# JuliaRobotics/RigidBodyDynamics.jl

Measured on AMD Instinct MI355X. Metric: ABA dynamics! evals/sec (Atlas 30-DoF, batch), higher is better.
Workload: dtype f64

## Files before the change

### rigidbodydynamics.jl_amd/csrc/rbd_bank.hpp

```cpp
#pragma once

#ifndef RBD_BANK_WAVES
#define RBD_BANK_WAVES 2
#endif
#ifndef RBD_BANK_FK_LDS
#define RBD_BANK_FK_LDS 0
#endif
#ifndef RBD_BANK_HANDOFF_LDS
#define RBD_BANK_HANDOFF_LDS 0
#endif

#ifdef RBD_BANK_FIXED_NL
#define RBD_BANK_UNROLL _Pragma("unroll")
namespace rbd { constexpr int kBankNs[] = {RBD_BANK_FIXED_NS}; }
#define RBD_BK_NL RBD_BANK_FIXED_NL
#define RBD_BK_L0 RBD_BANK_FIXED_L0
#define RBD_BK_NS(l) kBankNs[l]
#ifdef RBD_BANK_FIXED_PERM
#define RBD_BK_PERM(l) (((RBD_BANK_FIXED_PERM) >> (l)) & 1ull)
#else
#define RBD_BK_PERM(l) (kBankNs[l] > 1)
#endif
#else
#define RBD_BANK_UNROLL _Pragma("unroll 1")
#define RBD_BK_NL M.nlevels
#define RBD_BK_L0 M.L0
#define RBD_BK_NS(l) ns_next(nss, M.ns_desc)
#define RBD_BK_PERM(l) ((M.perm_down >> (l)) & 1)
#endif

namespace rbd {

template <typename T> struct alignas(2 * sizeof(T)) Pair2 { T a, b; };

RBD_DEV void wave_lds_sync() {
  __builtin_amdgcn_fence(__ATOMIC_RELEASE, "wavefront");
  __builtin_amdgcn_wave_barrier();
  __builtin_amdgcn_fence(__ATOMIC_ACQUIRE, "wavefront");
}


#define RBD_MASSIGN6(MOV)                                                                                                              \
  unsigned long long sv;                                                                                                               \
  asm volatile("s_and_saveexec_b64 %[sv], %[mk]\n\t" MOV " %[d0], %[s0]\n\t" MOV " %[d1], %[s1]\n\t" MOV " %[d2], %[s2]\n\t" MOV          \
               " %[d3], %[s3]\n\t" MOV " %[d4], %[s4]\n\t" MOV " %[d5], %[s5]\n\ts_mov_b64 exec, %[sv]\n\ts_nop 0"                         \
               : [sv] "=&s"(sv), [d0] "+v"(d[0]), [d1] "+v"(d[1]), [d2] "+v"(d[2]), [d3] "+v"(d[3]), [d4] "+v"(d[4]), [d5] "+v"(d[5])    \
               : [mk] "s"(mask), [s0] "v"(s[0]), [s1] "v"(s[1]), [s2] "v"(s[2]), [s3] "v"(s[3]), [s4] "v"(s[4]), [s5] "v"(s[5])          \
               : "scc")
RBD_DEV void massign6(unsigned long long mask, double* d, const double* s) { RBD_MASSIGN6("v_mov_b64"); }
RBD_DEV void massign6(unsigned long long mask, float* d, const float* s) { RBD_MASSIGN6("v_mov_b32"); }
template <typename T, int N> RBD_DEV void massign(bool m, T* d, const T* s) {
  static_assert(N % 6 == 0, "blocks of 6");
  const unsigned long long mask = __builtin_amdgcn_ballot_w64(m);
#pragma unroll
  for (int k = 0; k < N; k += 6) massign6(mask, d + k, s + k);
}

enum { PK_KIN = 0, PK_FWD = 6, PARK_PAIRS = 16, PK_XCH = 16, XCH_PAIRS = 14, BANK_LDS_PAIRS = PARK_PAIRS + XCH_PAIRS };

template <typename T, int N> RBD_DEV void lds_put(Pair2<T>* col, int pair0, const T* x) {
#pragma unroll
  for (int i = 0; i < (N + 1) / 2; ++i) {
    Pair2<T> v;
    v.a = x[2 * i];
    v.b = (2 * i + 1 < N) ? x[2 * i + 1] : T(0);
    col[(pair0 + i) * 256] = v;
  }
}
template <typename T, int N> RBD_DEV void lds_get(const Pair2<T>* col, int pair0, T* x) {
#pragma unroll
  for (int i = 0; i < (N + 1) / 2; ++i) {
    const Pair2<T> v = col[(pair0 + i) * 256];
    x[2 * i] = v.a;
    if (2 * i + 1 < N) x[2 * i + 1] = v.b;
  }
}

__host__ __device__ constexpr int sym_row(int e) { return e < 6 ? 0 : e < 11 ? 1 : e < 15 ? 2 : e < 18 ? 3 : e < 20 ? 4 : 5; }
__host__ __device__ constexpr int sym_col(int e) { return e - SI(sym_row(e), sym_row(e)) + sym_row(e); }

template <typename T> struct BankRegs {
  Body<T> b;
  const T* rb;
  int pcol;
  T K[24];
  RBD_DEV T* R() { return K; }
  RBD_DEV T* p() { return K + 9; }
  RBD_DEV T* Tw() { return K + 12; }
  RBD_DEV T* vJ() { return K + 18; }
  T S[6], cb[6], IA[21], pA[6], U[6], Dinv, u;
  T tj[6];
  T acc[6], vd[6];
};

template <typename T> RBD_DEV void load_bank_body(const BankModel& M, int k, long B, Body<T>& b) {
  const int tid = blockIdx.x * blockDim.x + threadIdx.x;
  b.lane = threadIdx.x & 63;
  const long wave = tid >> 6;
  const int lps = M.lps;
  b.sub = b.lane & (lps - 1);
  b.base = b.lane - b.sub;
  b.state = wave * (64 / lps) + (b.lane / lps);
  b.valid = (b.sub < M.nbk[k]) && (b.state < B);
  const int4* ib4 = reinterpret_cast<const int4*>(M.ib[k] + (b.sub < M.nbk[k] ? b.sub : 0) * IB_STRIDE);
  const int4 w0 = ib4[0], w1 = ib4[1], w2 = ib4[2], w3 = ib4[3];
  static_assert(IB_PARENT == 0 && IB_JTYPE == 1 && IB_QOFF == 2 && IB_VOFF == 3 && IB_LEVEL == 4 && IB_NCHILD == 5 && IB_ORIG == 6 && IB_CHILD0 == 7 &&
                IB_MAXCHILD == 8 && IB_FLAGS == 15 && IB_STRIDE == 16, "record layout");
  b.parent = w0.x; b.jtype = w0.y; b.qoff = w0.z; b.voff = w0.w;
  b.level = b.valid ? w1.x : -1;
  b.nchild = w1.y; b.orig = w1.z;
  b.child[0] = w1.w; b.child[1] = w2.x; b.child[2] = w2.y; b.child[3] = w2.z; b.child[4] = w2.w; b.child[5] = w3.x; b.child[6] = w3.y; b.child[7] = w3.z;
  b.flags = w3.w;
  b.plane = b.parent >= 0 ? b.base + b.parent : b.lane;
}

template <typename T, bool SIMPLE>
RBD_DEV void bank_fk_commit(bool mine, BankRegs<T>& c, const T* k18 , const T* XR, const T* Xp, const T* tl) {
  const T* pR = k18;
  const T* pp = k18 + 9;
  const T* pT = k18 + 12;
  T n[24];
  matmul3(pR, XR, n);
  matvec3(pR, Xp, n + 9);
#pragma unroll
  for (int k = 0; k < 3; ++k) n[9 + k] += pp[k];
  if (SIMPLE) {
    T S[6];
    matvec3(n, tl, S);
    cross3(n + 9, S, S + 3);
#pragma unroll
    for (int k = 0; k < 6; ++k) n[12 + k] = pT[k] + S[k] * tl[3];
    massign<T, 18>(mine, c.K, n);
  } else {
    xmotion(n, n + 9, tl, n + 18);
#pragma unroll
    for (int k = 0; k < 6; ++k) n[12 + k] = pT[k] + n[18 + k];
    massign<T, 24>(mine, c.K, n);
  }
}
template <typename T, bool SIMPLE> RBD_DEV void bank_fk_step(const BankModel& M, int l, bool perm, BankRegs<T>& c, Pair2<T>* lds, const T* XR, const T* Xp, const T* tl) {
  T k18[18];
  if (RBD_BANK_FK_LDS || perm) {
    if (c.b.level == l - 1 && c.b.nchild >= 1) {
      RBD_KEEP_BRANCH();
      lds_put<T, 18>(lds + threadIdx.x, PK_XCH, c.K);
    }
    wave_lds_sync();
    lds_get<T, 18>(lds + c.pcol, PK_XCH, k18);
    wave_lds_sync();
  } else {
#pragma unroll
    for (int k = 0; k < 18; ++k) k18[k] = from_prev_lane(c.K[k]);
  }
  bank_fk_commit<T, SIMPLE>(c.b.level == l, c, k18, XR, Xp, tl);
}
template <typename T, bool SIMPLE> RBD_DEV void bank_fk_cross(int L0, BankRegs<T>& c, const Pair2<T>* lds, const T* XR, const T* Xp, const T* tl) {
  T k18[18];
  lds_get<T, 18>(lds + c.pcol, PK_KIN, k18);
  bank_fk_commit<T, SIMPLE>(c.b.level == L0, c, k18, XR, Xp, tl);
}

// ... 69 lines not shown
        for (int k = 0; k < 6; ++k) tk.pA[k] += x[21 + k];
      }
    }
    wave_lds_sync();
  }
}

template <typename T> RBD_DEV void bank_joint_accel(bool mine, BankRegs<T>& r, const T* a_parent) {
  T ap[6], n[6];
#pragma unroll
  for (int k = 0; k < 6; ++k) ap[k] = a_parent[k] + r.cb[k];
  const T x = r.Dinv * (r.u - dot6(r.U, ap));
#pragma unroll
  for (int k = 0; k < 6; ++k) n[k] = ap[k] + r.S[k] * x;
  massign<T, 6>(mine, r.acc, n);
  r.vd[0] = mine ? x : r.vd[0];
}
template <typename T> RBD_DEV void bank_accel_step(const BankModel& M, int l, bool perm, BankRegs<T>& c, Pair2<T>* lds) {
  T ap[6];
  if (RBD_BANK_FK_LDS || perm) {
    if (c.b.level == l - 1 && c.b.nchild >= 1) {
      RBD_KEEP_BRANCH();
      lds_put<T, 6>(lds + threadIdx.x, PK_XCH, c.acc);
    }
    wave_lds_sync();
    lds_get<T, 6>(lds + c.pcol, PK_XCH, ap);
    wave_lds_sync();
  } else {
#pragma unroll
    for (int k = 0; k < 6; ++k) ap[k] = from_prev_lane(c.acc[k]);
  }
  bank_joint_accel(c.b.level == l, c, ap);
}

#ifdef RBD_PROFILE_PHASES
__device__ long long rbd_bank_phase_clock[16];
#define RBD_MARK(i) do { if (blockIdx.x == 0 && threadIdx.x == 0) rbd_bank_phase_clock[i] = clock64(); } while (0)
#else
#define RBD_MARK(i)
#endif

template <typename T, bool R> struct InPtr { typedef const T* type; };
template <typename T> struct InPtr<T, true> { typedef const T* __restrict__ type; };

template <typename T, bool FUSED, bool SIMPLE>
RBD_DEV void aba_bank_body(const BankModel& M, long B, typename InPtr<T, !FUSED>::type q, typename InPtr<T, !FUSED>::type v, const T* __restrict__ tau,
                           const T* __restrict__ fext, T* __restrict__ vdot, T* __restrict__ qdot, Layout Lq, Layout Lv, Layout Lf, const MkFuse& F,
                           Pair2<T>* const lds) {
  Pair2<T>* const col = lds + threadIdx.x;
  RBD_MARK(0);
  BankRegs<T> r0, r1;
  auto fetch = [&](int k, BankRegs<T>& c, T* qj, T* vj) {
    load_bank_body(M, k, B, c.b);
    c.rb = reinterpret_cast<const T*>(M.rb[k]) + (c.b.sub < M.nbk[k] ? c.b.sub : 0) * RB_STRIDE;
    c.pcol = (int)threadIdx.x - c.b.sub + (c.b.parent >= 0 ? c.b.parent : c.b.sub);
    if (SIMPLE) {
      const bool fl = c.b.jtype == RBD_JOINT_QUAT_FLOATING;
      const long sc = c.b.state < B ? c.b.state : B - 1;
      const T* qp = q + ((long)c.b.qoff * Lq.sk + sc * Lq.sb);
      const long va = (long)c.b.voff * Lv.sk + sc * Lv.sb;
      const bool hv = v != nullptr, ht = tau != nullptr;
      qj[0] = qp[0];
      vj[0] = hv ? v[va] : T(0);
      c.tj[0] = ht ? tau[va] : T(0);
#pragma unroll
      for (int k2 = 1; k2 < 7; ++k2) qj[k2] = T(0);
#pragma unroll
      for (int k2 = 1; k2 < 6; ++k2) { vj[k2] = T(0); c.tj[k2] = T(0); }
      if (fl) {
        RBD_KEEP_BRANCH();
#pragma unroll
        for (int k2 = 1; k2 < 7; ++k2) qj[k2] = qp[k2 * Lq.sk];
        if (hv) {
#pragma unroll
          for (int k2 = 1; k2 < 6; ++k2) vj[k2] = v[va + k2 * Lv.sk];
        }
        if (ht) {
#pragma unroll
          for (int k2 = 1; k2 < 6; ++k2) c.tj[k2] = tau[va + k2 * Lv.sk];
        }
      }
    } else {
      load_joint_q(c.b, q, Lq, qj);
      load_joint_v(c.b, v, Lv, vj);
      load_joint_v(c.b, tau, Lv, c.tj);
    }
  };
  auto setup = [&](BankRegs<T>& c, T* qj, T* vj, T* XR, T* Xp, T* tl, T* ta ) {
    if (SIMPLE) {
      const bool fl = c.b.jtype == RBD_JOINT_QUAT_FLOATING;
      const T ax[3] = {c.rb[RB_AXIS], c.rb[RB_AXIS + 1], c.rb[RB_AXIS + 2]};
      T Rj[9], pj[3] = {T(0), T(0), T(0)};
      T sn, cs;
      ta[0] = ax[0]; ta[1] = ax[1]; ta[2] = ax[2]; ta[3] = vj[0];
      sincos_fast(qj[0], &sn, &cs);
      rot_axis_sc(ax, sn, cs, Rj);
#pragma unroll
      for (int k = 0; k < 3; ++k) { tl[k] = ax[k] * vj[0]; tl[3 + k] = T(0); }
      if (fl) {
        RBD_KEEP_BRANCH();
        rot_quat(qj[0], qj[1], qj[2], qj[3], Rj);
        pj[0] = qj[4]; pj[1] = qj[5]; pj[2] = qj[6];
#pragma unroll
        for (int k = 0; k < 6; ++k) tl[k] = vj[k];
        if (qdot != nullptr && c.b.valid) {
          const T w = qj[0], x = qj[1], y = qj[2], z = qj[3];
          T o[7];
// ... 54 lines not shown
      se3_comm(c.Tw(), c.S, c.cb);
#pragma unroll
      for (int i = 0; i < 6; ++i) c.cb[i] *= c.K[18];
    } else {
      se3_comm(c.Tw(), c.vJ(), c.cb);
    }
    RInertia<T> I;
    T Jb[6], mc[3], fe[6];
#pragma unroll
    for (int i = 0; i < 6; ++i) Jb[i] = c.rb[RB_J + i];
#pragma unroll
    for (int i = 0; i < 3; ++i) mc[i] = c.rb[RB_MC + i];
    inertia_to_root(Jb, mc, c.rb[RB_M], c.R(), c.p(), I);
    T Io[21], po[6];
    sym6_from_inertia(I, Io);
    momentum_cross(I, c.Tw(), po);
    load_body_wrench(c.b, fext, Lf, fe);
#pragma unroll
    for (int i = 0; i < 21; ++i) c.IA[i] = accumulate ? c.IA[i] + Io[i] : Io[i];
#pragma unroll
    for (int i = 0; i < 6; ++i) c.pA[i] = accumulate ? c.pA[i] + (po[i] - fe[i]) : po[i] - fe[i];
#pragma unroll
    for (int i = 0; i < 6; ++i) c.U[i] = T(0);
    c.Dinv = T(0);
    c.u = T(0);
    if (floating) xforce(c.R(), c.p(), c.tj, c.U);
  };

  T qj0[7], vj0[6], qj1[7], vj1[6];
  fetch(0, r0, qj0, vj0);
  fetch(1, r1, qj1, vj1);
  if (FUSED) {
    if (F.close_prev) {
      mk_stage_lane(r0.b, 4, (T)F.dt, qj0, vj0, (const T*)nullptr, F.W, (T*)F.q_state, (T*)F.v_state, Lq, Lv);
      mk_stage_lane(r1.b, 4, (T)F.dt, qj1, vj1, (const T*)nullptr, F.W, (T*)F.q_state, (T*)F.v_state, Lq, Lv);
    }
    mk_stage_lane(r0.b, F.stage, (T)F.dt, qj0, vj0, (const T*)nullptr, F.W, (T*)F.q_state, (T*)F.v_state, Lq, Lv);
    mk_stage_lane(r1.b, F.stage, (T)F.dt, qj1, vj1, (const T*)nullptr, F.W, (T*)F.q_state, (T*)F.v_state, Lq, Lv);
    pd_control_lane(r0.b, F, Lq, qj0, vj0, r0.tj);
    pd_control_lane(r1.b, F, Lq, qj1, vj1, r1.tj);
  }
  {
    T XR[9], Xp[3], tl[6], ta[4];
    setup(r0, qj0, vj0, XR, Xp, tl, ta);
    RBD_MARK(1);
RBD_BANK_UNROLL
    for (int l = 1; l < RBD_BK_L0; ++l) bank_fk_step<T, SIMPLE>(M, l, RBD_BK_PERM(l), r0, lds, XR, Xp, SIMPLE ? ta : tl);
  }
  {
    T XR[9], Xp[3], tl[6], ta[4];
    RBD_MARK(2);
    setup(r1, qj1, vj1, XR, Xp, tl, ta);
    RBD_MARK(3);
    lds_put<T, (SIMPLE ? 20 : 24)>(col, PK_KIN, r0.K);
    wave_lds_sync();
    bank_fk_cross<T, SIMPLE>(RBD_BK_L0, r1, lds, XR, Xp, SIMPLE ? ta : tl);
RBD_BANK_UNROLL
    for (int l = RBD_BK_L0 + 1; l < RBD_BK_NL; ++l) bank_fk_step<T, SIMPLE>(M, l, RBD_BK_PERM(l), r1, lds, XR, Xp, SIMPLE ? ta : tl);
  }
  RBD_MARK(4);
  terms(r1, false);
  RBD_MARK(5);

  NsStream nss = ns_begin(M.ns_desc);
  (void)nss;
RBD_BANK_UNROLL
  for (int l = RBD_BK_NL - 1; l > RBD_BK_L0; --l) {
    bank_finish_joint<T, SIMPLE>(l, r1);
    bank_handoff<T, RBD_BANK_HANDOFF_LDS>(l, RBD_BK_NS(l), r1, r1, lds);
  }
  bank_finish_joint<T, SIMPLE>(RBD_BK_L0, r1);
  RBD_MARK(6);
#pragma unroll
  for (int i = 0; i < 21; ++i) r0.IA[i] = T(0);
#pragma unroll
  for (int i = 0; i < 6; ++i) r0.pA[i] = T(0);
  bank_handoff<T, 1>(RBD_BK_L0, RBD_BK_NS(RBD_BK_L0), r1, r0, lds);
  {
    lds_get<T, (SIMPLE ? 20 : 24)>(col, PK_KIN, r0.K);
    T f20[20];
#pragma unroll
    for (int i = 0; i < 6; ++i) { f20[i] = r1.U[i]; f20[8 + i] = r1.S[i]; f20[14 + i] = r1.cb[i]; }
    f20[6] = r1.Dinv;
    f20[7] = r1.u;
    lds_put<T, 20>(col, PK_FWD, f20);
  }
  RBD_MARK(7);
  terms(r0, true);
  RBD_MARK(8);
RBD_BANK_UNROLL
  for (int l = RBD_BK_L0 - 1; l >= 1; --l) {
    bank_finish_joint<T, SIMPLE>(l, r0);
    bank_handoff<T, RBD_BANK_HANDOFF_LDS>(l, RBD_BK_NS(l), r0, r0, lds);
  }
  bank_finish_joint<T, SIMPLE>(0, r0);
  RBD_MARK(9);

#pragma unroll
  for (int i = 0; i < 6; ++i) { r0.acc[i] = T(0); r0.vd[i] = T(0); }
  {
    const T a0[6] = {T(0), T(0), T(0), T(-M.gravity[0]), T(-M.gravity[1]), T(-M.gravity[2])};
    BankRegs<T>& c = r0;
    const bool fl0 = c.b.level == 0 && c.b.jtype == RBD_JOINT_QUAT_FLOATING;
    T fa[6] = {T(0), T(0), T(0), T(0), T(0), T(0)}, fv[6] = {T(0), T(0), T(0), T(0), T(0), T(0)};
    if (fl0) {
      RBD_KEEP_BRANCH();
      T rhs[6], d[6], k12[12];
#pragma unroll
      for (int i = 0; i < 6; ++i) rhs[i] = c.U[i] - c.pA[i];
      sym6_solve(c.IA, rhs, fa);
#pragma unroll
      for (int i = 0; i < 6; ++i) d[i] = fa[i] - a0[i];
      lds_get<T, 12>(col, PK_KIN, k12);
      xmotion_inv(k12, k12 + 9, d, fv);
    }
    massign<T, 6>(fl0, c.acc, fa);
    massign<T, 6>(fl0, c.vd, fv);
    bank_joint_accel(c.b.level == 0 && !fl0, c, a0);
  }
RBD_BANK_UNROLL
  for (int l = 1; l < RBD_BK_L0; ++l) bank_accel_step<T>(M, l, RBD_BK_PERM(l), r0, lds);
  RBD_MARK(10);
  if (vdot) store_joint_v(r0.b, vdot, Lv, r0.vd);
  if (FUSED) store_joint_v(r0.b, (T*)F.W.vd[F.stage], Lv, r0.vd);
  {
    T f20[20];
    lds_get<T, 20>(col, PK_FWD, f20);
#pragma unroll
    for (int i = 0; i < 6; ++i) {
      r1.U[i] = f20[i];
      r1.S[i] = f20[8 + i];
      r1.cb[i] = f20[14 + i];
      r1.acc[i] = T(0);
      r1.vd[i] = T(0);
    }
    r1.Dinv = f20[6];
    r1.u = f20[7];
  }
  {
    lds_put<T, 6>(col, PK_XCH, r0.acc);
    wave_lds_sync();
    T ap[6];
    lds_get<T, 6>(lds + r1.pcol, PK_XCH, ap);
    wave_lds_sync();
    bank_joint_accel(r1.b.level == RBD_BK_L0, r1, ap);
  }
RBD_BANK_UNROLL
  for (int l = RBD_BK_L0 + 1; l < RBD_BK_NL; ++l) bank_accel_step<T>(M, l, RBD_BK_PERM(l), r1, lds);
  RBD_MARK(11);
  if (vdot) store_joint_v(r1.b, vdot, Lv, r1.vd);
  if (FUSED) store_joint_v(r1.b, (T*)F.W.vd[F.stage], Lv, r1.vd);
}
#ifndef RBD_BANK_FIXED_NL
template <typename T, bool FUSED, bool SIMPLE>
__global__ __launch_bounds__(256, RBD_BANK_WAVES) void aba_bank_kernel(BankModel M, long B, typename InPtr<T, !FUSED>::type q, typename InPtr<T, !FUSED>::type v,
                                                         const T* __restrict__ tau, const T* __restrict__ fext, T* __restrict__ vdot,
                                                         T* __restrict__ qdot, Layout Lq, Layout Lv, Layout Lf, MkFuse F) {
  extern __shared__ double bank_lds_raw[];
  aba_bank_body<T, FUSED, SIMPLE>(M, B, q, v, tau, fext, vdot, qdot, Lq, Lv, Lf, F, reinterpret_cast<Pair2<T>*>(bank_lds_raw));
}
#endif

enum { RNEA_LDS_PAIRS = 12 };
template <typename T> struct RneaRegs {
  Body<T> b;
  const T* rb;
  int pcol;
  T K[24], w[6];
  RBD_DEV T* R() { return K; }
  RBD_DEV T* p() { return K + 9; }
  RBD_DEV T* Tw() { return K + 12; }
  RBD_DEV T* acc() { return K + 18; }
};

template <typename T, bool SIMPLE>
RBD_DEV void rnea_fk_commit(bool mine, RneaRegs<T>& c, const T* k24, const T* XR, const T* Xp, const T* tl, const T* al) {
  const T* pR = k24;
  const T* pp = k24 + 9;
// ... 24 lines not shown
template <typename T, bool SIMPLE>
RBD_DEV void rnea_fk_step(const BankModel& M, int l, bool perm, RneaRegs<T>& c, Pair2<T>* lds, const T* XR, const T* Xp, const T* tl, const T* al) {
  T k24[24];
  if (perm) {
    if (c.b.level == l - 1 && c.b.nchild >= 1) {
      RBD_KEEP_BRANCH();
      lds_put<T, 24>(lds + threadIdx.x, 0, c.K);
    }
    wave_lds_sync();
    lds_get<T, 24>(lds + c.pcol, 0, k24);
    wave_lds_sync();
  } else {
#pragma unroll
    for (int k = 0; k < 24; ++k) k24[k] = from_prev_lane(c.K[k]);
  }
  rnea_fk_commit<T, SIMPLE>(c.b.level == l, c, k24, XR, Xp, tl, al);
}

template <typename T, bool CROSS> RBD_DEV void rnea_gather(int l, int ns, const RneaRegs<T>& gv, RneaRegs<T>& tk) {
  const bool takes = (tk.b.level == l - 1);
  if (!CROSS) {
    T t[6];
#pragma unroll
    for (int k = 0; k < 6; ++k) t[k] = from_next_lane(gv.w[k]);
    if (takes && tk.b.nchild >= 1) {
      RBD_KEEP_BRANCH();
#pragma unroll
      for (int k = 0; k < 6; ++k) tk.w[k] += t[k];
    }
  }
#pragma unroll 1
  for (int s = CROSS ? 0 : 1; s < ns; ++s) {
    const bool take = takes && (s < tk.b.nchild);
    const int src = take ? tk.b.base + child_sel(tk.b, s) : tk.b.lane;
    T t[6];
#pragma unroll
    for (int k = 0; k < 6; ++k) t[k] = shfl(gv.w[k], src);
    if (take) {
      RBD_KEEP_BRANCH();
#pragma unroll
      for (int k = 0; k < 6; ++k) tk.w[k] += t[k];
    }
  }
}

template <typename T, bool SIMPLE>
RBD_DEV void rnea_bank_body(const BankModel& M, long B, int ncol, const T* __restrict__ q, const T* __restrict__ v, const T* __restrict__ vdot,
                            const T* __restrict__ fext, T* __restrict__ tau, T* __restrict__ qdot, Layout Lq, Layout Lv, Layout Lf, T* __restrict__ acc_out,
                            T* __restrict__ jw_out, Pair2<T>* const lds) {
  RneaRegs<T> r0, r1;
  const bool out_vec = store6_vec(acc_out ? acc_out : jw_out, Lf, (int)sizeof(T)) && store6_vec(jw_out ? jw_out : acc_out, Lf, (int)sizeof(T));
  auto fetch = [&](int k, RneaRegs<T>& c, T* qj, T* vj, T* aj) {
    load_bank_body(M, k, B, c.b);
    c.rb = reinterpret_cast<const T*>(M.rb[k]) + (c.b.sub < M.nbk[k] ? c.b.sub : 0) * RB_STRIDE;
    c.pcol = (int)threadIdx.x - c.b.sub + (c.b.parent >= 0 ? c.b.parent : c.b.sub);
    if (SIMPLE) {
      const bool fl = c.b.jtype == RBD_JOINT_QUAT_FLOATING;
      const long sc = c.b.state < B ? c.b.state : B - 1;
      const T* qp = q + ((long)c.b.qoff * Lq.sk + sc * Lq.sb);
      const long va = (long)c.b.voff * Lv.sk + sc * Lv.sb;
      const bool hv = v != nullptr, ha = vdot != nullptr;
      qj[0] = qp[0];
      vj[0] = hv ? v[va] : T(0);
      aj[0] = ha ? vdot[va] : T(0);
#pragma unroll
      for (int k2 = 1; k2 < 7; ++k2) qj[k2] = T(0);
#pragma unroll
      for (int k2 = 1; k2 < 6; ++k2) { vj[k2] = T(0); aj[k2] = T(0); }
      if (fl) {
        RBD_KEEP_BRANCH();
#pragma unroll
        for (int k2 = 1; k2 < 7; ++k2) qj[k2] = qp[k2 * Lq.sk];
        if (hv) {
#pragma unroll
          for (int k2 = 1; k2 < 6; ++k2) vj[k2] = v[va + k2 * Lv.sk];
        }
        if (ha) {
#pragma unroll
          for (int k2 = 1; k2 < 6; ++k2) aj[k2] = vdot[va + k2 * Lv.sk];
        }
      }
    } else {
      load_joint_q(c.b, q, Lq, qj);
      load_joint_v(c.b, v, Lv, vj);
      load_joint_v(c.b, vdot, Lv, aj);
    }
  };
  auto setup = [&](RneaRegs<T>& c, const T* qj, const T* vj, const T* aj, T* XR, T* Xp, T* tl, T* al, T* ta) {
    if (SIMPLE) {
      const bool fl = c.b.jtype == RBD_JOINT_QUAT_FLOATING;
      const T ax[3] = {c.rb[RB_AXIS], c.rb[RB_AXIS + 1], c.rb[RB_AXIS + 2]};
      ta[0] = ax[0]; ta[1] = ax[1]; ta[2] = ax[2]; ta[3] = vj[0]; ta[4] = aj[0];
      T Rj[9], pj[3] = {T(0), T(0), T(0)}, sn, cs;
      sincos_fast(qj[0], &sn, &cs);
      rot_axis_sc(ax, sn, cs, Rj);
#pragma unroll
      for (int k = 0; k < 3; ++k) { tl[k] = ax[k] * vj[0]; tl[3 + k] = T(0); al[k] = ax[k] * aj[0]; al[3 + k] = T(0); }
      if (fl) {
        RBD_KEEP_BRANCH();
        rot_quat(qj[0], qj[1], qj[2], qj[3], Rj);
        pj[0] = qj[4]; pj[1] = qj[5]; pj[2] = qj[6];
#pragma unroll
        for (int k = 0; k < 6; ++k) { tl[k] = vj[k]; al[k] = aj[k]; }
        if (qdot != nullptr && c.b.valid) {
          const T w = qj[0], x = qj[1], y = qj[2], z = qj[3];
          T o[7];
          o[0] = (-x * vj[0] - y * vj[1] - z * vj[2]) * T(0.5);
// ... 120 lines not shown
```

### rigidbodydynamics.jl_amd/csrc/rbd_capi.hip

```cpp
#include <hip/hip_runtime.h>
#include <chrono>
#include <climits>
#include <cmath>
#include <unistd.h>

#include <algorithm>
#include <cstdio>
#include <cstdlib>
#include <cstring>
#include <new>
#include <string>
#include <vector>

#include "rbd_hip.h"
#include "rbd_internal.hpp"
#include "rbd_chain_plan.hpp"
#include "rbd_track_plan.hpp"
#include "rbd_walk_plan.hpp"
#include "rbd_reroot.hpp"
#include "rbd_state_plan.hpp"
#include "rbd_jit.hpp"
#include "rbd_mk_fuse.hpp"
#include "rbd_tangent.hpp"
#include "rbd_tangent_mk.hpp"
// ... 1094 lines not shown
  if (*have >= need) return RBD_OK;
  if (*p) HIP_TRY(hipFree(*p));
  *p = nullptr; *have = 0;
  HIP_TRY(hipMalloc(p, need));
  *have = need;
  return RBD_OK;
}

class HostIO {
 public:
  HostIO(rbd_ws* w, int memory) : w_(w), host_(memory == RBD_MEM_HOST) {}
  int in(const void* src, size_t bytes, const void** dev) {
    void* d;
    const int st = stage(const_cast<void*>(src), bytes, true, false, &d);
    *dev = d;
    return st;
  }
  int out(void* dst, size_t bytes, void** dev) { return stage(dst, bytes, false, true, dev); }
  int inout(void* buf, size_t bytes, void** dev) { return stage(buf, bytes, true, true, dev); }
  int finish() {
    for (int k = 0; k < nout_; ++k) HIP_TRY(hipMemcpyAsync(out_[k].host, out_[k].dev, out_[k].bytes, hipMemcpyDeviceToHost, w_->stream));
    return RBD_OK;
  }

 private:
  enum { kSlots = sizeof(rbd_ws::stage) / sizeof(void*) };
  struct Out { void* host; const void* dev; size_t bytes; };
  int stage(void* buf, size_t bytes, bool copy_in, bool copy_out, void** dev) {
    *dev = buf;
    if (!host_ || !buf) return RBD_OK;
    const int k = nslot_++;
    if (k >= kSlots) return RBD_ERR_INVALID_ARGUMENT;
    if (int st = ensure(&w_->stage[k], &w_->stage_bytes[k], bytes)) return st;
    *dev = w_->stage[k];
    if (copy_in && bytes) HIP_TRY(hipMemcpyAsync(*dev, buf, bytes, hipMemcpyHostToDevice, w_->stream));
    if (copy_out) out_[nout_++] = Out{buf, *dev, bytes};
    return RBD_OK;
  }
  rbd_ws* w_;
  bool host_;
  int nslot_ = 0, nout_ = 0;
  Out out_[kSlots];
};

}

static int bank_simple(const rbd_model* m) {
  for (int i = 0; i < m->nb; ++i)
    if (m->jt_ref[i] != RBD_JOINT_REVOLUTE && !(m->jt_ref[i] == RBD_JOINT_QUAT_FLOATING && m->parent_ref[i] < 0)) return 0;
  return 1;
}
static std::string bank_program_source(const rbd_model* m, int dtype, int simple) {
  if (m->bank_lps <= 0) return std::string();
  return spec_bank_source(m->nlevels, m->bank_L0, m->nslots.data(), (unsigned long long)m->bank_perm_down, simple, dtype);
}
static std::string loop_program_source(const rbd_model* m, int dtype, std::vector<int32_t>* xi_store) {
  if (!m->loop_fused_ok) return std::string();
  xi_store->assign(3 * (size_t)m->nb, 0);
  for (int i = 0; i < m->nb; ++i) { (*xi_store)[3 * i] = m->parent_ref[i]; (*xi_store)[3 * i + 1] = m->qoff_ref[i]; (*xi_store)[3 * i + 2] = m->slot_of[i]; }
  LoopTables L{m->nb, m->nq, m->nv, m->nc, m->nloops, &m->loop_i, &m->loop_path, &m->jt_ref, &m->voff_ref, xi_store, &m->loop_r, &m->axis_ref, &m->axis2_ref, &m->rb, m->gravity};
  return spec_loop_source(L, dtype);
}
static bool walk_tables(const rbd_model* m, bool rerooted, WalkTables* W) {
  const TrackPlan* P; const WalkPlan* K;
  if (rerooted) { if (!m->rrs.ok || !m->rrs.track.ok || !m->rrs.walk.ok) return false; P = &m->rrs.track; K = &m->rrs.walk; }
  else { if (!m->track.ok || !m->walk.ok) return false; P = &m->track; K = &m->walk; }
  *W = WalkTables{};
  W->ns = P->ns; W->G = P->G; W->nA = P->nA; W->nB = P->nB; W->nS = K->nS; W->nq = m->nq; W->nv = m->nv; W->flt = P->has_floating; W->gen = P->general; W->rr = rerooted;
  W->ri = &P->ri; W->wk = &K->wk; W->rrc = &P->rr;
  W->mk1 = &m->mk1; W->mkf = &m->mkf;
  for (int k = 0; k < 5; ++k) { W->sfm[k] = 0; for (int s2 = 0; s2 < P->ns; ++s2) W->sfm[k] |= (uint64_t)((P->sf[s2] >> k) & 1) << s2; }
  if (rerooted) {
    W->nchain = (int)(m->rr.chain_i.size() / RC_I_STRIDE); W->fq = m->rr.fq; W->fv = m->rr.fv; W->chain_i = &m->rr.chain_i; W->chain_r = &m->rr.chain_r; W->fXp = m->rr.fXp;
    if (W->nchain < 1) return false;
  }
  return true;
}
static bool walk_program_rerooted(const rbd_model* m, int dtype, int pair) {
  WalkTables W;
  return tune("walk_no_reroot", 0) == 0 && walk_tables(m, true, &W) && walk_lds_bytes(W.ns, W.G, W.nq, W.nv, W.nA, W.nB, W.nS, (dtype == RBD_F64 || pair) ? 8 : 4, dtype == RBD_F64 ? 8 : 4) <= 160 * 1024;
}
static std::string walk_program_source(const rbd_model* m, int dtype, bool rerooted, int kind, int pair) {
  WalkTables W;
  if (!walk_tables(m, rerooted, &W)) return std::string();
  return walk_spec_source(W, dtype, kind, pair);
}
static bool capturing(rbd_ws* w);
template <class Source>
static hipModule_t spec_module(rbd_ws* w, SpecSlot& p, Source source, bool walk, bool wait, const char* fallback) {
  if (p.tried) return nullptr;
  if (!jit_available()) { p.tried = true; return nullptr; }
  if (capturing(w)) return nullptr;
  if (p.src.empty()) p.src = source();
  if (p.src.empty()) { p.tried = true; return nullptr; }
  std::string log;
  std::vector<char> code;
  const int js = code_object_get(p.src, walk, wait, &code, &log);
  if (js == JIT_PENDING) return nullptr;
  p.tried = true;
  std::string src;
  src.swap(p.src);
  if (js == JIT_FAILED || code.empty()) { g_last_hip_error = std::string("run-time compilation failed (") + fallback + "): " + log; return nullptr; }
  if (hipModuleLoadData(&p.mod, code.data()) != hipSuccess) { (void)hipGetLastError(); p.mod = nullptr; jit_cache_discard(src); return nullptr; }
  return p.mod;
}
static const int kNoScratchCheck = INT_MAX;
static hipFunction_t spec_kernel(hipModule_t mod, const char* name, int max_scratch, int* scratch = nullptr) {
// ... 1796 lines not shown
```

### rigidbodydynamics.jl_amd/csrc/rbd_jit.hip

```cpp
#include <dlfcn.h>
#include <hip/hip_runtime.h>
#include <hip/hiprtc.h>
#include <sys/stat.h>
#include <unistd.h>

#include <cstdio>
#include <cstdlib>
#include <algorithm>
#include <cstring>
#include <atomic>
#include <map>
#include <memory>
#include <mutex>
#include <thread>
#include <string>
#include <vector>

#include "rbd_internal.hpp"
#include "rbd_jit.hpp"
#include "rbd_walk_plan.hpp"
#include "rbd_jit_embed.inc"

namespace rbd {

// ... 466 lines not shown
    s += "extern \"C\" __global__ __launch_bounds__(64, RBD_SPEC_CHOL_WAVES) void chol_spec_nom_f32(long B, const float* Mg, const float* tau, const float* c, float* x, rbd::Layout Lv,\n"
         "                                                                       int* notpd, float* Mcopy, rbd::Layout Lc) {\n"
         "  rbd::spec::chol_spec<false, false>(B, blockIdx.x, Mg, tau, c, x, Lv, notpd, nullptr, Lc, nullptr);\n}\n";
    s += "extern \"C\" __global__ __launch_bounds__(64, RBD_SPEC_CHOL_WAVES) void chol_spec_packed_f32(long B, const float* Mg, const float* tau, const float* c, float* x, rbd::Layout Lv,\n"
         "                                                                          int* notpd, float* Mcopy, rbd::Layout Lc) {\n"
         "  __shared__ __align__(16) float mst[rbd::spec::chol_emit_lds()];\n"
         "  rbd::spec::chol_spec<true, true>(B, blockIdx.x, Mg, tau, c, x, Lv, notpd, Mcopy, Lc, mst);\n}\n";
  }
  if (emit) {
    snprintf(b, sizeof b, "extern \"C\" __global__ __launch_bounds__(64, 2) void emit_spec_%s(long B, const %s* Mg, %s* Mcopy, rbd::Layout Lc) {\n"
                          "  __shared__ __align__(16) %s mst[16 * rbd::spec::emit_mst<%s>()];\n  rbd::spec::emit_spec<%s>(B, blockIdx.x, Mg, Mcopy, Lc, mst);\n}\n", sfx, T, T, T, T, T);
    s += b;
  }
  return s;
}

std::string spec_loop_source(const LoopTables& L, int dtype) {
  if (!(L.nloops > 0 && L.nb <= 4 && L.nv <= 4 && L.nc <= 6 && L.nv < L.nc)) return std::string();
  const char* T = dtype == RBD_F32 ? "float" : "double";
  const char* sfx = dtype == RBD_F32 ? "f32" : "f64";
  std::string s;
  char b[1024];
  s += "// generated by rbd_jit.hip: the loop tables of one small mechanism as constants (rbd_loop_small.hpp)\n#include \"rbd_loop_small.hpp\"\nnamespace rbd_loop_plan {\n";
  auto ints = [&](const char* name, const std::vector<int32_t>& v) {
    snprintf(b, sizeof b, "__device__ const int32_t %s[%d] = ", name, (int)std::max<size_t>(v.size(), 1));
    s += b;
    if (v.empty()) s += "{0}"; else put_ints(s, v.data(), (int)v.size());
    s += ";\n";
  };
  auto reals = [&](const char* name, const std::vector<double>& v) {
    snprintf(b, sizeof b, "__device__ const %s %s[%d] = ", T, name, (int)std::max<size_t>(v.size(), 1));
    s += b;
    if (v.empty()) s += "{0}"; else put_reals(s, v.data(), (int)v.size());
    s += ";\n";
  };
  ints("LI", *L.li); ints("PATH", *L.path); ints("JT", *L.jt); ints("VOFF", *L.voff); ints("XI", *L.xi);
  reals("LR", *L.lr); reals("AXIS", *L.axis); reals("AXIS2", *L.axis2); reals("RB", *L.rb);
  snprintf(b, sizeof b, "struct View {\n  static constexpr int nloops = %d, nc = %d, nv = %d, nb = %d;\n", L.nloops, L.nc, L.nv, L.nb);
  s += b;
  snprintf(b, sizeof b, "  const int32_t* li = LI; const %s* lr = LR; const int32_t* path = PATH; const int32_t* jt = JT; const int32_t* voff = VOFF;\n"
                        "  const %s* axis = AXIS; const %s* axis2 = AXIS2; const int32_t* xi = XI; const %s* rb = RB; const %s* gains = nullptr;\n};\n}  // namespace rbd_loop_plan\n", T, T, T, T, T);
  s += b;
  snprintf(b, sizeof b, "extern \"C\" __global__ __launch_bounds__(64) void loop_spec_%s(long B, int stabilize, const %s* q, const %s* v, const %s* tau, const %s* fext,\n"
                        "    %s* Mg, %s* cg, %s* vdot, %s* qdot, %s* lambda, %s* Kg, %s* kg, rbd::Layout Lq, rbd::Layout Lm, rbd::Layout Lv, rbd::Layout Lf, rbd::Layout Lc,\n"
                        "    rbd::Layout Lk, int* notpd, const %s* gains) {\n", sfx, T, T, T, T, T, T, T, T, T, T, T, T);
  s += b;
  s += "  const long st = (long)blockIdx.x * blockDim.x + threadIdx.x;\n  if (st >= B) return;\n  rbd_loop_plan::View V;\n  V.gains = gains;  // nullptr: the model's gains, compile-time constants\n";
  snprintf(b, sizeof b, "  rbd::loop_fused_small_state<%s, rbd_loop_plan::View, %d, %d, %d, true>(V, st, stabilize, q, v, tau, fext, Mg, Mg, cg, vdot, qdot, lambda, Kg, kg,\n"
                        "      Lq, Lm, Lv, Lf, Lc, Lk, %.17g, %.17g, %.17g, notpd);\n}\n", T, L.nb, L.nv, L.nc, L.gravity[0], L.gravity[1], L.gravity[2]);
  s += b;
  return s;
}

std::string spec_bank_source(int nlevels, int L0, const int32_t* nslots, unsigned long long perm_down, int simple, int dtype) {
  if (nlevels < 2 || nlevels > 64 || L0 < 1 || L0 >= nlevels) return std::string();
  const char* T = dtype == RBD_F32 ? "float" : "double";
  const char* sfx = dtype == RBD_F32 ? "f32" : "f64";
  const char* SI = simple ? "true" : "false";
  std::string s;
  char b[1600];
  s += "// generated by rbd_jit.hip: the level structure of one mechanism for the banked kernels (aba_bank_body / rnea_bank_body, rbd_bank.hpp): loops over the levels unrolled,\n"
       "// DPP hop or exchange column and the number of later children known per level\n";
  snprintf(b, sizeof b, "#define RBD_BANK_FIXED_NL %d\n#define RBD_BANK_FIXED_L0 %d\n#define RBD_BANK_FIXED_PERM 0x%llxull\n#define RBD_BANK_FIXED_NS ", nlevels, L0, perm_down);
  s += b;
  for (int l = 0; l < nlevels; ++l) { snprintf(b, sizeof b, "%s%d", l ? "," : "", (int)nslots[l]); s += b; }
  s += "\n#include \"rbd_lane.hpp\"\n#include \"rbd_bank.hpp\"\n";
  const char* lds = "  __shared__ __align__(16) unsigned char lds[(size_t)rbd::BANK_LDS_PAIRS * 256 * sizeof(rbd::Pair2<%s>)];\n";
  for (int fused = 0; fused < 2; ++fused) {
    snprintf(b, sizeof b, "extern \"C\" __global__ __launch_bounds__(256, RBD_BANK_WAVES) void aba_bank_%sspec_%s(rbd::BankModel M, long B, const %s* q, const %s* v, const %s* tau,\n"
                          "    const %s* fext, %s* vdot, %s* qdot, rbd::Layout Lq, rbd::Layout Lv, rbd::Layout Lf, rbd::MkFuse F) {\n",
             fused ? "fused_" : "", sfx, T, T, T, T, T, T);
    s += b;
    snprintf(b, sizeof b, lds, T);
    s += b;
    snprintf(b, sizeof b, "  rbd::aba_bank_body<%s, %s, %s>(M, B, q, v, tau, fext, vdot, qdot, Lq, Lv, Lf, F, reinterpret_cast<rbd::Pair2<%s>*>(lds));\n}\n", T, fused ? "true" : "false", SI, T);
    s += b;
  }
  snprintf(b, sizeof b, "extern \"C\" __global__ __launch_bounds__(256, 2) void rnea_bank_spec_%s(rbd::BankModel M, long B, int ncol, const %s* q, const %s* v, const %s* vdot, const %s* fext,\n"
                        "    %s* tau, %s* qdot, rbd::Layout Lq, rbd::Layout Lv, rbd::Layout Lf, %s* acc_out, %s* jw_out) {\n"
                        "  __shared__ __align__(16) unsigned char lds[(size_t)rbd::RNEA_LDS_PAIRS * 256 * sizeof(rbd::Pair2<%s>)];\n"
                        "  rbd::rnea_bank_body<%s, %s>(M, B, ncol, q, v, vdot, fext, tau, qdot, Lq, Lv, Lf, acc_out, jw_out, reinterpret_cast<rbd::Pair2<%s>*>(lds));\n}\n",
           sfx, T, T, T, T, T, T, T, T, T, T, SI, T);
  s += b;
  return s;
}

size_t walk_spec_lds_bytes(const WalkTables& W, int dtype, int pair) {
  return walk_rows(W.nq, W.nv, W.nA, W.nB, W.nS) * WR_STRIDE * ((dtype == RBD_F64 || pair) ? 8 : 4);
}
bool walk_spec_has(int dtype, int ns, int G, size_t lds_rows_bytes) {
  return (dtype == RBD_F64 || dtype == RBD_F32) && ns >= 1 && ns <= WALK_MAX_STEPS && G >= 1 && G <= 4 && lds_rows_bytes <= 160 * 1024;
}
const char* walk_spec_suffix(int dtype, int pair) { return dtype == RBD_F64 ? "f64" : pair ? "f32x2" : "f32"; }
std::string walk_spec_source(const WalkTables& W, int dtype, int kind, int pair) {
  if (dtype == RBD_F64) pair = 0;
  const size_t lds = walk_spec_lds_bytes(W, dtype, pair);
  if (!walk_spec_has(dtype, W.ns, W.G, lds)) return std::string();
  const char* S = dtype == RBD_F64 ? "double" : "float";
  const char* T = dtype == RBD_F64 ? "double" : pair ? "rbd::f2" : "float";
  const char* sfx = walk_spec_suffix(dtype, pair);
  std::string s;
  char b[1400];
  {
    const char* e = getenv("RBD_TUNE"); const char* k = e ? strstr(e, "spec_variant=") : nullptr;
    if (k && (atol(k + 13) & 32)) s += "#define RBD_WALK_ABLATE_OUT_LOCAL 1\n";
    if (k && (atol(k + 13) & 256)) s += "#define RBD_WALK_NO_STAGE 1\n";
  }
  if (kind == 2) {
    snprintf(b, sizeof b, "// rbd-walk-sim-loop stash-from=a%d\n// rbd-jit-option: -mllvm\n// rbd-jit-option: -disable-machine-licm\n",
             256 - ((dtype == RBD_F64 || pair) ? 2 : 1) * W.ns * WALK_STASH_N);
    s += b;
  }
  s += "// generated by rbd_jit.hip: the walk plan of one mechanism as constants (aba_walk_spec / rnea_walk_spec, rbd_walk.hpp)\n#include \"rbd_walk.hpp\"\nnamespace rbd_walk_tables {\n";
  const int nrec = W.ns * W.G;
  snprintf(b, sizeof b, "__device__ const int32_t RI[%d] __attribute__((aligned(16))) = ", nrec * TI_STRIDE);
  s += b; put_ints(s, W.ri->data(), nrec * TI_STRIDE); s += ";\n";
  snprintf(b, sizeof b, "__device__ const %s RR[%d] = ", S, nrec * TR_STRIDE);
  s += b; put_reals(s, W.rrc->data(), nrec * TR_STRIDE); s += ";\n";
  snprintf(b, sizeof b, "__device__ const int32_t WK[%d] = ", nrec);
  s += b; put_ints(s, W.wk->data(), nrec); s += ";\n";
  const int nch = W.rr ? W.nchain : 0;
  snprintf(b, sizeof b, "__device__ const int32_t CHI[%d] = ", std::max(nch, 1) * 4);
// ... 334 lines not shown
```

### rigidbodydynamics.jl_amd/csrc/rbd_jit.hpp

```cpp
#pragma once
#include <cstdint>
#include <string>
#include <vector>

#include "rbd_state_plan.hpp"

namespace rbd {
bool jit_available();
enum { SPEC_MASS = 0, SPEC_ABA = 1, SPEC_RNEA = 2, SPEC_FAMILIES = 3 };
enum { SPEC_KIN = 11, SPEC_SLOTS = 4 };
inline int spec_slot(int family) { return family == SPEC_KIN ? 3 : family; }
bool spec_has(int family, int dtype, int nb, int nq, int nv, int n3 = 0);
bool spec_has_chol(int dtype, int nv);
std::string spec_source(const StatePlan& P, int nb, int nq, int nv, const uint64_t* row_mask, const double* gravity, int dtype, int family);
struct LoopTables {
  int nb, nq, nv, nc, nloops;
  const std::vector<int32_t>*li, *path, *jt, *voff, *xi;
  const std::vector<double>*lr, *axis, *axis2, *rb;
  const double* gravity;
};
std::string spec_loop_source(const LoopTables& L, int dtype);
std::string spec_bank_source(int nlevels, int L0, const int32_t* nslots, unsigned long long perm_down, int simple, int dtype);
struct WalkTables {
  int ns, G, nA, nB, nS, nq, nv, flt, gen, rr;
  const std::vector<int32_t>*ri, *wk;
  const std::vector<double>* rrc;
  uint64_t sfm[5];
  int nchain, fq, fv;
  const std::vector<int32_t>* chain_i;
  const std::vector<double>* chain_r;
  const double* fXp;
  const std::vector<int32_t>*mk1, *mkf;
};
bool walk_spec_has(int dtype, int ns, int G, size_t lds_rows_bytes);
size_t walk_spec_lds_bytes(const WalkTables& W, int dtype, int pair = 0);
const char* walk_spec_suffix(int dtype, int pair);
std::string walk_spec_source(const WalkTables& W, int dtype, int kind = 0, int pair = 0);
enum { JIT_READY = 0, JIT_PENDING = 1, JIT_FAILED = 2 };
bool jit_async();
void jit_wait_idle();
int jit_code_object_get(const std::string& source, bool wait, std::vector<char>* code, std::string* log);
int jit_walk_code_object_get(const std::string& source, bool wait, std::vector<char>* code, std::string* log);
int jit_kd_cover_agprs(std::vector<char>* code);
bool jit_walk_admit(const std::string& source, std::vector<char>* code, std::string* log);
std::vector<char> jit_walk_code_object(const std::string& source, std::string* log);
std::vector<char> jit_code_object(const std::string& source, std::string* log);
void jit_cache_discard(const std::string& source);
}
```

Baseline: 217.6 million.

## Keep bank ABA state in registers and bake per-lane joint tables into JIT kernel

New measurement: 213.7 million (median of 2 runs). 1.8% lower.

```diff
diff --git a/rigidbodydynamics.jl_amd/csrc/rbd_bank.hpp b/rigidbodydynamics.jl_amd/csrc/rbd_bank.hpp
--- a/rigidbodydynamics.jl_amd/csrc/rbd_bank.hpp
+++ b/rigidbodydynamics.jl_amd/csrc/rbd_bank.hpp
@@ -29,9 +29,30 @@
 #define RBD_BK_PERM(l) ((M.perm_down >> (l)) & 1)
 #endif
 
+#ifdef RBD_BANK_FIXED_QV0
+#define RBD_BK_LPS RBD_BANK_FIXED_LPS
+#define RBD_BK_NBK(k) ((k) ? RBD_BANK_FIXED_NBK1 : RBD_BANK_FIXED_NBK0)
+#else
+#define RBD_BK_LPS M.lps
+#define RBD_BK_NBK(k) M.nbk[k]
+#endif
+#ifdef RBD_BANK_FIXED_REGPARK
+#define RBD_BK_REGPARK 1
+#else
+#define RBD_BK_REGPARK 0
+#endif
+
 namespace rbd {
 
 template <typename T> struct alignas(2 * sizeof(T)) Pair2 { T a, b; };
+
+#ifdef RBD_BANK_FIXED_QV0
+constexpr unsigned kBankQV[2][RBD_BANK_FIXED_LPS] = {{RBD_BANK_FIXED_QV0}, {RBD_BANK_FIXED_QV1}};
+template <int K, int LO, int N> RBD_DEV unsigned bank_qv_sel(int sub) {
+  if constexpr (N == 1) return kBankQV[K][LO];
+  else return (sub & (N / 2)) ? bank_qv_sel<K, LO + N / 2, N / 2>(sub) : bank_qv_sel<K, LO, N / 2>(sub);
+}
+#endif
 
 RBD_DEV void wave_lds_sync() {
   __builtin_amdgcn_fence(__ATOMIC_RELEASE, "wavefront");
@@ -56,7 +77,11 @@
   for (int k = 0; k < N; k += 6) massign6(mask, d + k, s + k);
 }
 
+#if RBD_BK_REGPARK
+enum { PK_KIN = 0, PK_FWD = 0, PARK_PAIRS = 0, PK_XCH = 0, XCH_PAIRS = 14, BANK_LDS_PAIRS = XCH_PAIRS };
+#else
 enum { PK_KIN = 0, PK_FWD = 6, PARK_PAIRS = 16, PK_XCH = 16, XCH_PAIRS = 14, BANK_LDS_PAIRS = PARK_PAIRS + XCH_PAIRS };
+#endif
 
 template <typename T, int N> RBD_DEV void lds_put(Pair2<T>* col, int pair0, const T* x) {
 #pragma unroll
@@ -81,7 +106,11 @@
 
 template <typename T> struct BankRegs {
   Body<T> b;
+#if RBD_BK_REGPARK
+  T rb[RB_STRIDE];
+#else
   const T* rb;
+#endif
   int pcol;
   T K[24];
   RBD_DEV T* R() { return K; }
@@ -97,16 +126,22 @@
   const int tid = blockIdx.x * blockDim.x + threadIdx.x;
   b.lane = threadIdx.x & 63;
   const long wave = tid >> 6;
-  const int lps = M.lps;
+  const int lps = RBD_BK_LPS;
   b.sub = b.lane & (lps - 1);
   b.base = b.lane - b.sub;
   b.state = wave * (64 / lps) + (b.lane / lps);
-  b.valid = (b.sub < M.nbk[k]) && (b.state < B);
-  const int4* ib4 = reinterpret_cast<const int4*>(M.ib[k] + (b.sub < M.nbk[k] ? b.sub : 0) * IB_STRIDE);
+  b.valid = (b.sub < RBD_BK_NBK(k)) && (b.state < B);
+  const int4* ib4 = reinterpret_cast<const int4*>(M.ib[k] + (b.sub < RBD_BK_NBK(k) ? b.sub : 0) * IB_STRIDE);
   const int4 w0 = ib4[0], w1 = ib4[1], w2 = ib4[2], w3 = ib4[3];
   static_assert(IB_PARENT == 0 && IB_JTYPE == 1 && IB_QOFF == 2 && IB_VOFF == 3 && IB_LEVEL == 4 && IB_NCHILD == 5 && IB_ORIG == 6 && IB_CHILD0 == 7 &&
                 IB_MAXCHILD == 8 && IB_FLAGS == 15 && IB_STRIDE == 16, "record layout");
   b.parent = w0.x; b.jtype = w0.y; b.qoff = w0.z; b.voff = w0.w;
+#ifdef RBD_BANK_FIXED_QV0
+  {
+    const unsigned qv = k ? bank_qv_sel<1, 0, RBD_BANK_FIXED_LPS>(b.sub) : bank_qv_sel<0, 0, RBD_BANK_FIXED_LPS>(b.sub);
+    b.qoff = (int)(qv & 0xfffu); b.voff = (int)((qv >> 12) & 0xfffu); b.jtype = (int)(qv >> 24);
+  }
+#endif
   b.level = b.valid ? w1.x : -1;
   b.nchild = w1.y; b.orig = w1.z;
   b.child[0] = w1.w; b.child[1] = w2.x; b.child[2] = w2.y; b.child[3] = w2.z; b.child[4] = w2.w; b.child[5] = w3.x; b.child[6] = w3.y; b.child[7] = w3.z;
@@ -282,7 +317,15 @@
   BankRegs<T> r0, r1;
   auto fetch = [&](int k, BankRegs<T>& c, T* qj, T* vj) {
     load_bank_body(M, k, B, c.b);
-    c.rb = reinterpret_cast<const T*>(M.rb[k]) + (c.b.sub < M.nbk[k] ? c.b.sub : 0) * RB_STRIDE;
+#if RBD_BK_REGPARK
+    {
+      const T* __restrict__ rbp = reinterpret_cast<const T*>(M.rb[k]) + (c.b.sub < RBD_BK_NBK(k) ? c.b.sub : 0) * RB_STRIDE;
+#pragma unroll
+      for (int i = 0; i < RB_STRIDE; ++i) c.rb[i] = rbp[i];
+    }
+#else
+    c.rb = reinterpret_cast<const T*>(M.rb[k]) + (c.b.sub < RBD_BK_NBK(k) ? c.b.sub : 0) * RB_STRIDE;
+#endif
     c.pcol = (int)threadIdx.x - c.b.sub + (c.b.parent >= 0 ? c.b.parent : c.b.sub);
     if (SIMPLE) {
       const bool fl = c.b.jtype == RBD_JOINT_QUAT_FLOATING;
@@ -443,9 +486,10 @@
     RBD_MARK(2);
     setup(r1, qj1, vj1, XR, Xp, tl, ta);
     RBD_MARK(3);
-    lds_put<T, (SIMPLE ? 20 : 24)>(col, PK_KIN, r0.K);
+    lds_put<T, (RBD_BK_REGPARK ? 18 : SIMPLE ? 20 : 24)>(col, PK_KIN, r0.K);
     wave_lds_sync();
     bank_fk_cross<T, SIMPLE>(RBD_BK_L0, r1, lds, XR, Xp, SIMPLE ? ta : tl);
+    if (RBD_BK_REGPARK) wave_lds_sync();
 RBD_BANK_UNROLL
     for (int l = RBD_BK_L0 + 1; l < RBD_BK_NL; ++l) bank_fk_step<T, SIMPLE>(M, l, RBD_BK_PERM(l), r1, lds, XR, Xp, SIMPLE ? ta : tl);
   }
@@ -467,7 +511,7 @@
 #pragma unroll
   for (int i = 0; i < 6; ++i) r0.pA[i] = T(0);
   bank_handoff<T, 1>(RBD_BK_L0, RBD_BK_NS(RBD_BK_L0), r1, r0, lds);
-  {
+  if (!RBD_BK_REGPARK) {
     lds_get<T, (SIMPLE ? 20 : 24)>(col, PK_KIN, r0.K);
     T f20[20];
 #pragma unroll
@@ -502,7 +546,12 @@
       sym6_solve(c.IA, rhs, fa);
 #pragma unroll
       for (int i = 0; i < 6; ++i) d[i] = fa[i] - a0[i];
-      lds_get<T, 12>(col, PK_KIN, k12);
+      if (RBD_BK_REGPARK) {
+#pragma unroll
+        for (int i = 0; i < 12; ++i) k12[i] = c.K[i];
+      } else {
+        lds_get<T, 12>(col, PK_KIN, k12);
+      }
       xmotion_inv(k12, k12 + 9, d, fv);
     }
     massign<T, 6>(fl0, c.acc, fa);
@@ -514,7 +563,10 @@
   RBD_MARK(10);
   if (vdot) store_joint_v(r0.b, vdot, Lv, r0.vd);
   if (FUSED) store_joint_v(r0.b, (T*)F.W.vd[F.stage], Lv, r0.vd);
-  {
+  if (RBD_BK_REGPARK) {
+#pragma unroll
+    for (int i = 0; i < 6; ++i) { r1.acc[i] = T(0); r1.vd[i] = T(0); }
+  } else {
     T f20[20];
     lds_get<T, 20>(col, PK_FWD, f20);
 #pragma unroll
@@ -645,7 +697,7 @@
   const bool out_vec = store6_vec(acc_out ? acc_out : jw_out, Lf, (int)sizeof(T)) && store6_vec(jw_out ? jw_out : acc_out, Lf, (int)sizeof(T));
   auto fetch = [&](int k, RneaRegs<T>& c, T* qj, T* vj, T* aj) {
     load_bank_body(M, k, B, c.b);
-    c.rb = reinterpret_cast<const T*>(M.rb[k]) + (c.b.sub < M.nbk[k] ? c.b.sub : 0) * RB_STRIDE;
+    c.rb = reinterpret_cast<const T*>(M.rb[k]) + (c.b.sub < RBD_BK_NBK(k) ? c.b.sub : 0) * RB_STRIDE;
     c.pcol = (int)threadIdx.x - c.b.sub + (c.b.parent >= 0 ? c.b.parent : c.b.sub);
     if (SIMPLE) {
       const bool fl = c.b.jtype == RBD_JOINT_QUAT_FLOATING;
diff --git a/rigidbodydynamics.jl_amd/csrc/rbd_capi.hip b/rigidbodydynamics.jl_amd/csrc/rbd_capi.hip
--- a/rigidbodydynamics.jl_amd/csrc/rbd_capi.hip
+++ b/rigidbodydynamics.jl_amd/csrc/rbd_capi.hip
@@ -1170,7 +1170,8 @@
 }
 static std::string bank_program_source(const rbd_model* m, int dtype, int simple) {
   if (m->bank_lps <= 0) return std::string();
-  return spec_bank_source(m->nlevels, m->bank_L0, m->nslots.data(), (unsigned long long)m->bank_perm_down, simple, dtype);
+  const int32_t* ib[2] = {m->bank_ib[0].data(), m->bank_ib[1].data()};
+  return spec_bank_source(m->nlevels, m->bank_L0, m->nslots.data(), (unsigned long long)m->bank_perm_down, simple, dtype, m->bank_lps, m->bank_nb, ib);
 }
 static std::string loop_program_source(const rbd_model* m, int dtype, std::vector<int32_t>* xi_store) {
   if (!m->loop_fused_ok) return std::string();
diff --git a/rigidbodydynamics.jl_amd/csrc/rbd_jit.hip b/rigidbodydynamics.jl_amd/csrc/rbd_jit.hip
--- a/rigidbodydynamics.jl_amd/csrc/rbd_jit.hip
+++ b/rigidbodydynamics.jl_amd/csrc/rbd_jit.hip
@@ -542,7 +542,8 @@
   return s;
 }
 
-std::string spec_bank_source(int nlevels, int L0, const int32_t* nslots, unsigned long long perm_down, int simple, int dtype) {
+std::string spec_bank_source(int nlevels, int L0, const int32_t* nslots, unsigned long long perm_down, int simple, int dtype, int lps, const int32_t* nbk,
+                             const int32_t* const* ib) {
   if (nlevels < 2 || nlevels > 64 || L0 < 1 || L0 >= nlevels) return std::string();
   const char* T = dtype == RBD_F32 ? "float" : "double";
   const char* sfx = dtype == RBD_F32 ? "f32" : "f64";
@@ -554,10 +555,31 @@
   snprintf(b, sizeof b, "#define RBD_BANK_FIXED_NL %d\n#define RBD_BANK_FIXED_L0 %d\n#define RBD_BANK_FIXED_PERM 0x%llxull\n#define RBD_BANK_FIXED_NS ", nlevels, L0, perm_down);
   s += b;
   for (int l = 0; l < nlevels; ++l) { snprintf(b, sizeof b, "%s%d", l ? "," : "", (int)nslots[l]); s += b; }
-  s += "\n#include \"rbd_lane.hpp\"\n#include \"rbd_bank.hpp\"\n";
+  s += "\n#define RBD_BANK_FIXED_REGPARK 1\n";
+  bool packs = lps >= 1 && lps <= 64 && (lps & (lps - 1)) == 0 && nbk && ib && nbk[0] >= 1 && nbk[1] >= 1 && nbk[0] <= lps && nbk[1] <= lps;
+  for (int k = 0; k < 2 && packs; ++k)
+    for (int j = 0; j < nbk[k]; ++j) {
+      const int32_t* r = ib[k] + (size_t)j * IB_STRIDE;
+      packs = r[IB_QOFF] >= 0 && r[IB_QOFF] < 4096 && r[IB_VOFF] >= 0 && r[IB_VOFF] < 4096 && r[IB_JTYPE] >= 0 && r[IB_JTYPE] < 256;
+    }
+  if (packs) {
+    snprintf(b, sizeof b, "#define RBD_BANK_FIXED_LPS %d\n#define RBD_BANK_FIXED_NBK0 %d\n#define RBD_BANK_FIXED_NBK1 %d\n", lps, (int)nbk[0], (int)nbk[1]);
+    s += b;
+    for (int k = 0; k < 2; ++k) {
+      snprintf(b, sizeof b, "#define RBD_BANK_FIXED_QV%d ", k);
+      s += b;
+      for (int j = 0; j < lps; ++j) {
+        const int32_t* r = ib[k] + (size_t)(j < nbk[k] ? j : 0) * IB_STRIDE;
+        snprintf(b, sizeof b, "%s0x%xu", j ? "," : "", (unsigned)r[IB_QOFF] | (unsigned)r[IB_VOFF] << 12 | (unsigned)r[IB_JTYPE] << 24);
+        s += b;
+      }
+      s += "\n";
+    }
+  }
+  s += "#include \"rbd_lane.hpp\"\n#include \"rbd_bank.hpp\"\n";
   const char* lds = "  __shared__ __align__(16) unsigned char lds[(size_t)rbd::BANK_LDS_PAIRS * 256 * sizeof(rbd::Pair2<%s>)];\n";
   for (int fused = 0; fused < 2; ++fused) {
-    snprintf(b, sizeof b, "extern \"C\" __global__ __launch_bounds__(256, RBD_BANK_WAVES) void aba_bank_%sspec_%s(rbd::BankModel M, long B, const %s* q, const %s* v, const %s* tau,\n"
+    snprintf(b, sizeof b, "extern \"C\" __global__ __launch_bounds__(256, 1) void aba_bank_%sspec_%s(rbd::BankModel M, long B, const %s* q, const %s* v, const %s* tau,\n"
                           "    const %s* fext, %s* vdot, %s* qdot, rbd::Layout Lq, rbd::Layout Lv, rbd::Layout Lf, rbd::MkFuse F) {\n",
              fused ? "fused_" : "", sfx, T, T, T, T, T, T);
     s += b;
diff --git a/rigidbodydynamics.jl_amd/csrc/rbd_jit.hpp b/rigidbodydynamics.jl_amd/csrc/rbd_jit.hpp
--- a/rigidbodydynamics.jl_amd/csrc/rbd_jit.hpp
+++ b/rigidbodydynamics.jl_amd/csrc/rbd_jit.hpp
@@ -20,7 +20,8 @@
   const double* gravity;
 };
 std::string spec_loop_source(const LoopTables& L, int dtype);
-std::string spec_bank_source(int nlevels, int L0, const int32_t* nslots, unsigned long long perm_down, int simple, int dtype);
+std::string spec_bank_source(int nlevels, int L0, const int32_t* nslots, unsigned long long perm_down, int simple, int dtype, int lps, const int32_t* nbk,
+                             const int32_t* const* ib);
 struct WalkTables {
   int ns, G, nA, nB, nS, nq, nv, flt, gen, rr;
   const std::vector<int32_t>*ri, *wk;
```
